# yjb6/SaRO-GS

Measured on AMD Instinct MI355X. Metric: rendered views/s (fwd+bwd) at 1080p vs #Gaussians, higher is better.
Workload: dtype f32; 1 GPU; BASELINE configs[4] stress-1080p: synth(P=3000000, seed 0) SH3, 1920x1080, one view per GPU, fwd+bwd; protocol=SURVEY 8d: 1 / median of per-call device-synchronised wall-clock fwd+bwd, pose_table=off for value (every pose a first visit); on for value_warm, gaussians=3000000, width=1920, height=1080, sh_degree=3, exp_mode=0, poses_per_rank=8, late_gaussians_cold=2255988, word_fork=0

## Files before the change

### include/gsrast.h

```cpp
#ifndef GSRAST_H_INCLUDED
#define GSRAST_H_INCLUDED

#include <stddef.h>
#include <stdint.h>

#ifdef __cplusplus
extern "C" {
#endif

#define GSRAST_ABI_VERSION 6
#define GSRAST_TILE_X 16
#define GSRAST_TILE_Y 16

typedef void* (*gsrast_alloc_fn)(void* ctx, size_t bytes);

int gsrast_forward(gsrast_alloc_fn geometry_alloc, void* geometry_ctx,
                   gsrast_alloc_fn binning_alloc, void* binning_ctx,
                   gsrast_alloc_fn image_alloc, void* image_ctx,
                   int P, int D, int M,
                   const float* background,
                   int width, int height,
                   const float* means3D,
                   const float* shs,
                   const float* colors_precomp,
// ... 66 lines not shown

int gsrast_grad_rows_pack(int P, const unsigned char* touched , float* const* dense, const float* factor , uint32_t* rows, uint32_t cap, void* stream);
int gsrast_grad_rows_clear(int P, const uint32_t* chunks, int n_chunks, size_t chunk_words, uint32_t cap, float* const* dense , int M,
                           float* dL_dsh, float* d_features_dc, float* d_features_rest, void* stream);
int gsrast_grad_rows_add(int P, const uint32_t* chunk, uint32_t cap, float* const* dense, int D, int M, const float* means3D, float scale,
                         float* dL_dsh, float* d_features_dc, float* d_features_rest, void* stream);

int gsrast_debug_export(int P, int R, int width, int height,
                        const char* geom_buffer, const char* binning_buffer, const char* image_buffer,
                        float* depths, float* means2D , float* cov3D ,
                        float* conic_opacity , float* rgb ,
                        unsigned char* clamped , uint32_t* tiles_touched,
                        uint64_t* keys_sorted , uint32_t* point_list ,
                        uint32_t* ranges , float* final_T ,
                        uint32_t* n_contrib , void* stream);

typedef struct gsrast_options {
    int exp_mode;
    int binning;
    int tile_clip;
    int cull;
    int lpt;
    int speculative;
    int fwd_pixels_per_lane;
    int bwd_pixels_per_lane;
    int sh_grad_factors;
    int side_stream;
    int grads_zeroed;
    int backward_phase;
    int depth_sort;
// ... 298 lines not shown
```

### saro-gs_amd/csrc/gsrast_binning.h

```cpp
#pragma once
#include "gsrast_common.h"

namespace gsrast {
#define GSRAST_OCC_ATTR(n) __attribute__((amdgpu_waves_per_eu(n, n)))
#ifdef GSRAST_RSCAT_WAVES
#define GSRAST_RSCAT_OCC GSRAST_OCC_ATTR(GSRAST_RSCAT_WAVES)
#else
#define GSRAST_RSCAT_OCC
#endif
#ifdef GSRAST_BSCAT_WAVES
#define GSRAST_BSCAT_OCC GSRAST_OCC_ATTR(GSRAST_BSCAT_WAVES)
#else
#define GSRAST_BSCAT_OCC
#endif
#ifdef GSRAST_BSORT_WAVES
#define GSRAST_BSORT_OCC GSRAST_OCC_ATTR(GSRAST_BSORT_WAVES)
#else
#define GSRAST_BSORT_OCC
#endif
#ifdef GSRAST_EMIT_WAVES
#define GSRAST_EMIT_OCC GSRAST_OCC_ATTR(GSRAST_EMIT_WAVES)
#else
#define GSRAST_EMIT_OCC
#endif
// ... 772 lines not shown
    uint32_t run = wave_incl_scan(wsum) - wsum;
    const uint32_t wtot = __shfl(run + wsum, 63, 64);
#pragma unroll
    for (int d = 32; d >= 1; d >>= 1) { tsum += __shfl_xor(tsum, d, 64); wall += __shfl_xor(wall, d, 64); }
    uint32_t* scanbuf = reinterpret_cast<uint32_t*>(grp);
    for (uint32_t e = 0; e < E; e++) { const uint32_t t = lane * E + e; if (t < n) { run += aux[t]; scanbuf[t] = run; } }
    wave_sync();
    for (uint32_t t = lane; t < n; t += 64) bwincl[(size_t)b * BK_CAP + t] = scanbuf[t];
    if (lane == 0) {
        if (early_only) { binfo[b] = make_uint4(n, wtot, n_all - n, over); binfo_all[b] = make_uint4(n_all, wall, tsum, over); }
        else binfo[b] = make_uint4(n, wtot, tsum, over);
        bwsum[b] = wtot;
    }
}

__device__ __forceinline__ void depth_bucket_totals(const uint4* __restrict__ binfo, uint32_t nb, uint32_t* __restrict__ scalars,
                                                    uint32_t* host_out = nullptr, uint32_t host_seq = 0,
                                                    const uint4* __restrict__ binfo_e = nullptr )
{
    __shared__ unsigned long long s_t[256];
    __shared__ uint32_t s_q[256], s_qe[256];
    uint32_t over = 0, q = 0, qe = 0;
    unsigned long long tsum = 0;
    for (uint32_t k0 = threadIdx.x; k0 < nb; k0 += 256 * 8) {
        uint4 v[8];
#pragma unroll
        for (int u = 0; u < 8; u++) { const uint32_t k = k0 + u * 256; v[u] = k < nb ? binfo[k] : make_uint4(0u, 0u, 0u, 0u); }
#pragma unroll
        for (int u = 0; u < 8; u++) { q += v[u].y; tsum += v[u].z; over |= v[u].w; }
        if (binfo_e) {
// ... 119 lines not shown
        const uint32_t prev = tile_keys_sorted[i - 1];
        if (cur != prev) { ranges[prev].y = i; ranges[cur].x = i; }
    }
    if (i == R - 1) ranges[cur].y = R;
}

__device__ __forceinline__ double sqrt_newton(double x)
{
    const float xf = (float)x;
    if (!(xf > 1e-30f) || !(xf < 1e30f)) return sqrt(x);
    const float s0f = __builtin_sqrtf(xf);
    const double s0 = (double)s0f;
    return __builtin_fma(__builtin_fma(-s0, s0, x), 0.5 * (double)__builtin_amdgcn_rcpf(s0f), s0);
}

__global__ void __launch_bounds__(256) GSRAST_EMIT_OCC
emit_column_runs_kernel(int P, const uint32_t* __restrict__ order, const uint32_t* __restrict__ woffsets ,
                        const float4* __restrict__ binrec, int W, int H, int cull, uint32_t capQ,
                        uint16_t* __restrict__ run_keys, uint2* __restrict__ run_vals,
                        const uint4* __restrict__ binfo = nullptr, const uint32_t* __restrict__ bwsum = nullptr, uint32_t nbuckets = 0,
                        uint32_t* __restrict__ scalars = nullptr ,
                        uint32_t* __restrict__ host_out = nullptr, uint32_t host_seq = 0 ,
                        const uint4* __restrict__ binfo_all = nullptr, const uint32_t* __restrict__ pred = nullptr,
                        uint32_t* __restrict__ redo_bucket_cnt = nullptr, int n_redo_cnt = 0, HintTable* __restrict__ redo_hints = nullptr,
                        unsigned long long* __restrict__ host_fallback = nullptr, uint32_t host_fb_seq = 0 ,
                        const unsigned char* __restrict__ need2 = nullptr, int gx_tiles = 0, uint32_t* __restrict__ pass2_counts = nullptr,
                        const float4* __restrict__ rec0 = nullptr, const float4* __restrict__ rec1 = nullptr, const uint2* __restrict__ rect = nullptr)
{
    if (pred && *pred == 0u) return;
    __shared__ uint32_t s_e[4][64], s_g[4][64], s_x0[4][64], s_yh[4][64];
    __shared__ double s_det[4][64], s_t2c[4][64], s_invc[4][64], s_dymax[4][64], s_dxtop[4][64];
    __shared__ float s_b[4][64], s_mx[4][64], s_my[4][64];
    __shared__ uint32_t s_mode[4][64];
    if (redo_bucket_cnt && blockIdx.x == nbuckets) {
        for (int i = threadIdx.x; i < n_redo_cnt; i += blockDim.x) redo_bucket_cnt[i] = 0u;
        if (threadIdx.x == 0 && redo_hints) atomicAdd(&redo_hints->cut_fallbacks, 1u);
        uint32_t q2 = 1u;
        if (pass2_counts) {
            unsigned long long* const s_t2 = reinterpret_cast<unsigned long long*>(&s_det[0][0]);
            uint32_t* const s_q2 = &s_e[0][0];
            unsigned long long ts = 0; uint32_t q = 0;
            for (uint32_t k = threadIdx.x; k < nbuckets; k += 256) { const uint4 v = binfo[k]; q += v.y; ts += v.z; }
            s_t2[threadIdx.x] = ts; s_q2[threadIdx.x] = q;
            __syncthreads();
            for (int st = 128; st > 0; st >>= 1) { if ((int)threadIdx.x < st) { s_t2[threadIdx.x] += s_t2[threadIdx.x + st]; s_q2[threadIdx.x] += s_q2[threadIdx.x + st]; } __syncthreads(); }
            if (threadIdx.x == 0) { pass2_counts[0] = (uint32_t)s_t2[0]; pass2_counts[1] = s_q2[0]; pass2_counts[2] = 0u; pass2_counts[3] = (uint32_t)(s_t2[0] >> 32); q2 = s_q2[0] ? s_q2[0] : 1u; }
        }
        if (threadIdx.x == 0 && host_fallback) __hip_atomic_store(host_fallback, ((unsigned long long)host_fb_seq << 32) | (unsigned long long)q2, __ATOMIC_RELAXED, __HIP_MEMORY_SCOPE_SYSTEM);
        return;
    }
    const unsigned lane = lane_id(), wave = threadIdx.x >> 6;
    uint32_t nloc = 0, run0 = 0, nchunks = 1;
    uint32_t pre_g = 0, pre_w = 0, pre_wm = 0;
    if (binfo) {
        __shared__ uint32_t s_run0[4];
        uint32_t part = 0;
        const uint4* w4 = reinterpret_cast<const uint4*>(bwsum);
        if (scalars && blockIdx.x == 0) { depth_bucket_totals(binfo_all ? binfo_all : binfo, nbuckets, scalars, host_out, host_seq, binfo_all ? binfo : nullptr); return; }
        const uint32_t b = scalars ? blockIdx.x - 1u : blockIdx.x, n4 = (b + 3) / 4;
        order += (size_t)b * BK_CAP; woffsets += (size_t)b * BK_CAP;
        pre_g = order[threadIdx.x]; pre_w = woffsets[threadIdx.x]; pre_wm = threadIdx.x ? woffsets[threadIdx.x - 1] : 0u;
        for (uint32_t q0 = threadIdx.x; q0 < n4; q0 += 256 * 8) {
            uint4 v[8];
#pragma unroll
            for (int u = 0; u < 8; u++) { const uint32_t q = q0 + u * 256; v[u] = q < n4 ? w4[q] : make_uint4(0u, 0u, 0u, 0u); }
#pragma unroll
            for (int u = 0; u < 8; u++) {
                const uint32_t k = 4 * (q0 + u * 256);
                part += (k < b ? v[u].x : 0u) + (k + 1 < b ? v[u].y : 0u) + (k + 2 < b ? v[u].z : 0u) + (k + 3 < b ? v[u].w : 0u);
            }
        }
#pragma unroll
        for (int d = 32; d >= 1; d >>= 1) part += __shfl_xor(part, d, 64);
        if (lane == 0) s_run0[wave] = part;
        const uint4 bi = binfo[b];
        __syncthreads();
        run0 = s_run0[0] + s_run0[1] + s_run0[2] + s_run0[3];
        nloc = bi.x; nchunks = (nloc + 255u) / 256u;
        P = (int)nloc;
    }
    for (uint32_t chunk = 0; chunk < nchunks; chunk++) {
    if (chunk) __syncthreads();
    const int j = binfo ? (int)(chunk * 256u + threadIdx.x) : (int)(blockIdx.x * blockDim.x + threadIdx.x);
    uint32_t g = 0, w = 0, incl, x0 = 0, yh = 0;
    if (j < P) {
        const bool pre = binfo && chunk == 0;
        g = pre ? pre_g : order[j];
        incl = run0 + (pre ? pre_w : woffsets[j]);
        const uint32_t prev = j > 0 ? run0 + (pre ? pre_wm : woffsets[j - 1]) : run0;
        w = incl - prev;
        uint2 rc = make_uint2(0u, 0u);
        float4 r0 = make_float4(0.f, 0.f, 0.f, 0.f), r1 = r0;
        if (w != 0u) {
            if (binrec) {
                r0 = binrec[2 * (size_t)g]; r1 = binrec[2 * (size_t)g + 1];
                rc = make_uint2(__float_as_uint(r1.z), __float_as_uint(r1.w));
            } else {
// ... 63 lines not shown
            const int thi = min((int)(y0 + h) - 1, (int)fmin(phi, (double)(H - 1)) >> 4);
            if (empty || phi < 0.0 || plo > (double)(H - 1) || thi < tlo) h = 0;
            else { y0 = (uint32_t)tlo; h = (uint32_t)(thi - tlo + 1); }
            yhv = y0 | (h << 16);
        }
        if (need2 && (yhv >> 16) != 0u) {
            const uint32_t y0 = yhv & 0xFFFFu, h = yhv >> 16;
            bool any = false;
            for (uint32_t yy = y0; yy < y0 + h; yy++) any |= need2[yy * (uint32_t)gx_tiles + x] != 0;
            if (!any) yhv = y0;
        }
        run_keys[wstart + o] = (uint16_t)x;
        run_vals[wstart + o] = make_uint2(s_g[wave][sidx], yhv);
    }
    }
}

__global__ void __launch_bounds__(256)
run_hist_rows_kernel(const uint2* __restrict__ run_vals, uint32_t Q, const uint32_t* __restrict__ Q_dev,
                     uint32_t* __restrict__ block_hist, uint32_t nblk, uint32_t nrows ,
                     const uint32_t* __restrict__ pred = nullptr)
{
    __shared__ int diff[257];
    if (pred && *pred == 0u) return;
    Q = dev_count(Q, Q_dev);
    for (int k = threadIdx.x; k < 257; k += 256) diff[k] = 0;
    __syncthreads();
    const uint32_t r0 = blockIdx.x * RUNS_PER_BLOCK;
    for (uint32_t k = threadIdx.x; k < (uint32_t)RUNS_PER_BLOCK; k += 256) {
        const uint32_t r = r0 + k;
// ... 287 lines not shown
```

### saro-gs_amd/csrc/gsrast_capi.hip

```cpp
#include "gsrast_host.h"
#include "gsrast_common.h"
#include "gsrast_policy.h"
#include "gsrast_preprocess.h"
#include "gsrast_binning.h"
#include "gsrast_blend.h"
#include "gsrast_contrib.h"
#include "gsrast_features.h"
#include "gsrast_distort.h"
#include "gsrast_exchange.h"

#include <algorithm>
#include <atomic>
#include <chrono>
#include <cstdlib>
#include <thread>
#include <cstdio>
#include <cmath>
#include <cstring>
#include <dlfcn.h>
#ifndef GSRAST_LATE_FILL_WGS
#define GSRAST_LATE_FILL_WGS 256
#endif
#include <mutex>
#include <string>
// ... 814 lines not shown
    return v ? fail(GSRAST_E_ARG, "forward: a Gaussian passed as prefiltered was culled by the near plane (the reference traps: auxiliary.h:156-160)") : GSRAST_OK;
}

static const char* raw_inputs_check(int P, int M, const gsrast_raw_inputs* in)
{
    if (!in) return "raw: NULL inputs";
    if (P == 0) return nullptr;
    if (!in->xyz || !in->rotation || !in->scaling || !in->opacity_logit || !in->features_dc || (M > 1 && !in->features_rest)) return "raw: NULL required input";
    if (M < 1 || M * 3 > PP_SH_MAX || ((M * 3) & 3)) return "raw: M must be 4 or 16 (SH rows of a multiple of 16 bytes, at most 16 coefficients)";
    if (((uintptr_t)in->rotation | (uintptr_t)in->features_dc | (uintptr_t)in->features_rest | (uintptr_t)in->shs_res) & 15) return "raw: rotation / features_dc / features_rest / shs_res must be 16-byte aligned";
    return nullptr;
}

extern "C++" { namespace {
struct BucketSortArgs {
    const uint4* slab; const uint32_t* gcount; uint32_t nb; const uint32_t* bkey; uint32_t *border, *bwincl; uint4* binfo; uint32_t* bwsum;
    uint4* binfo_all = nullptr;
    const uint32_t* pred = nullptr; const unsigned long long* keep_bits = nullptr;
    uint32_t* zero_words = nullptr; uint32_t n_zero_words = 0; uint4* zero_quads = nullptr; uint32_t n_zero_quads = 0;
};
void launch_bucket_sort(hipStream_t s, const BucketSortArgs& a)
{
    depth_bucket_sort_kernel<<<(a.nb + BK_WAVES - 1) / BK_WAVES, 64 * BK_WAVES, 0, s>>>(a.slab, a.gcount, a.nb, a.bkey, a.border, a.bwincl, a.binfo, a.bwsum, a.binfo_all, a.pred, a.keep_bits,
                                                                                   a.zero_words, a.n_zero_words, a.zero_quads, a.n_zero_quads);
}
struct EmitArgs {
    uint32_t grid; int P; const uint32_t *order, *woffsets; const float4* binrec; int W, H, clip; uint32_t capQ; uint16_t* run_keys; uint2* run_vals;
    const float4 *rec0, *rec1; const uint2* rect;
    const uint4* binfo = nullptr; const uint32_t* bwsum = nullptr; uint32_t nbuckets = 0;
    uint32_t* scalars = nullptr; uint32_t* host_out = nullptr; uint32_t host_seq = 0;
    const uint4* binfo_all = nullptr; const uint32_t* pred = nullptr;
    uint32_t* redo_bucket_cnt = nullptr; int n_redo_cnt = 0; HintTable* redo_hints = nullptr; unsigned long long* host_fallback = nullptr; uint32_t host_fb_seq = 0;
    const unsigned char* need2 = nullptr; int gx_tiles = 0; uint32_t* pass2_counts = nullptr;
};
void launch_emit(hipStream_t s, const EmitArgs& a)
{
    emit_column_runs_kernel<<<a.grid, 256, 0, s>>>(a.P, a.order, a.woffsets, a.binrec, a.W, a.H, a.clip, a.capQ, a.run_keys, a.run_vals, a.binfo, a.bwsum, a.nbuckets, a.scalars,
                                               a.host_out, a.host_seq, a.binfo_all, a.pred, a.redo_bucket_cnt, a.n_redo_cnt, a.redo_hints, a.host_fallback, a.host_fb_seq,
                                               a.need2, a.gx_tiles, a.pass2_counts, a.rec0, a.rec1, a.rect);
}
bool trace_on() { static const bool on = getenv("GSRAST_TRACE") != nullptr; return on; }

struct ForwardRun {
    gsrast_context* const ctx; const gsrast_forward_call& c; const gsrast_options o; const std::chrono::steady_clock::time_point t_entry; const hipStream_t stream;
    ForwardPlan plan;
    const float *means3D, *shs, *opacities, *scales, *rotations;
    const gsrast_raw_inputs* rawin = nullptr; RawArgs raw{};
    float *out_acc_depth = nullptr, *out_alpha = nullptr;
    int P = 0, W = 0, H = 0; uint32_t T = 0, nbk = 0; CamArgs cam;
    GeomLayout GL; ImgLayout IL; char *geom = nullptr, *img = nullptr, *bin = nullptr; uint32_t cap = 0, capQ = 0;
    float4 *rec0, *rec1, *rec2, *binrec, *grec; uint32_t* tiles; uint2* rect; uint32_t *kA, *kB, *vA, *vB, *offsets, *woffsets, *hist, *scan_tmp, *scalars, *hint_sel, *prefilter_word;
    uint4 *bk_slab, *bk_info, *bk_info_e; uint32_t *bk_count, *bk_key, *bk_order, *bk_wincl, *bk_base, *bk_order_e, *bk_wincl_e, *bk_base_e;
    unsigned long long *color_skip, *cand_bits; unsigned char *untouched = nullptr, *tile_flags; uint32_t* bucket_cnt; uint16_t* bucket_list; uint2* ranges;
    uint32_t *zcut_used = nullptr, *tau_hist = nullptr, *zhist_call = nullptr; TauBins tau_bins{};
    HintTable* hints = nullptr;
    uint32_t zh_klo = 0, zh_wave_mask = 0; int zh_shift = 0;
    bool zhist_ctx = false; int tau_ctx_device = -1;
    struct SideJoinGuard {
        SideStream* side = nullptr; bool launched = false , joined = false;
        ~SideJoinGuard() { if (launched && side && !joined) (void)hipStreamSynchronize(side->stream); }
    } fork;
    bool bucketed = false;
    bool totals_pending = false;
    bool sort_redone = false;
    Readback *rb_pre = nullptr, *rb_flag = nullptr, *rb = nullptr; uint32_t *pre_alias = nullptr, *flag_alias = nullptr; uint32_t pre_seq = 0, flag_seq = 0;
    ChainGate* gate = nullptr; uint32_t gseq = 0, *gdone = nullptr, *gpred = nullptr;
    uint32_t counts[12] = { 0 }; uint32_t nQ1 = 0;
// ... 43 lines not shown
        GL = geom_layout((size_t)P);
        geom = (char*)c.geometry_alloc(c.geometry_ctx, GL.total);
        if (!geom) return fail(GSRAST_E_ALLOC, "forward: geometry allocation failed");
        IL = img_layout((size_t)W, (size_t)H);
        img = (char*)c.image_alloc(c.image_ctx, IL.total);
        if (!img) return fail(GSRAST_E_ALLOC, "forward: image allocation failed");
        rec0 = at<float4>(geom, GL.rec0); rec1 = at<float4>(geom, GL.rec1); rec2 = at<float4>(geom, GL.rec2); grec = at<float4>(geom, GL.grec);
        tiles = at<uint32_t>(geom, GL.tiles); rect = at<uint2>(geom, GL.rect);
        kA = at<uint32_t>(geom, GL.keyA); kB = at<uint32_t>(geom, GL.keyB); vA = at<uint32_t>(geom, GL.valA); vB = at<uint32_t>(geom, GL.valB);
        offsets = at<uint32_t>(geom, GL.offsets); woffsets = at<uint32_t>(geom, GL.woffsets); hist = at<uint32_t>(geom, GL.hist); scan_tmp = at<uint32_t>(geom, GL.scan_tmp);
        scalars = at<uint32_t>(geom, GL.scalars); hint_sel = scalars + HINT_SEL;
        bk_slab = at<uint4>(geom, GL.bk_slab); bk_info = at<uint4>(geom, GL.bk_info); bk_info_e = at<uint4>(geom, GL.bk_info_e);
        bk_count = at<uint32_t>(geom, GL.bk_count); bk_key = at<uint32_t>(geom, GL.bk_key);
        bk_order = at<uint32_t>(geom, GL.bk_order); bk_wincl = at<uint32_t>(geom, GL.bk_wincl); bk_base = at<uint32_t>(geom, GL.bk_base);
        bk_order_e = at<uint32_t>(geom, GL.bk_order_e); bk_wincl_e = at<uint32_t>(geom, GL.bk_wincl_e); bk_base_e = at<uint32_t>(geom, GL.bk_base_e);
        color_skip = at<unsigned long long>(geom, GL.color_skip); cand_bits = at<unsigned long long>(geom, GL.cand_bits);
        tile_flags = at<unsigned char>(img, IL.tile_flags); bucket_cnt = at<uint32_t>(img, IL.bucket_cnt); bucket_list = at<uint16_t>(img, IL.bucket_list);
        ranges = at<uint2>(img, IL.ranges);
        prefilter_word = c.prefiltered ? scalars + SC_PREFILTER : nullptr;
        if (prefilter_word) GS_HIP(hipMemsetAsync(prefilter_word, 0, sizeof(uint32_t), s));
        nbk = depth_buckets_host((size_t)P);
        zh_klo = ctx->zrange.klo.load(); zh_shift = ctx->zrange.shift.load();
        while ((((size_t)P + 63) / 64) / ((size_t)zh_wave_mask + 1) > 1024) zh_wave_mask = 2u * zh_wave_mask + 1u;
        if (o.side_stream) fork.side = side_stream_of(ctx);
        return GSRAST_OK;
    }

    int begin_policy(hipStream_t s)
    {
        hints = plan.want_hints ? hints_of(ctx, T, s) : nullptr;
// ... 72 lines not shown
                P, means3D, scales, rotations, opacities, raw, c.cov3D_precomp, cam, c.radii, rec0, rec1, cov_dbg,
                tiles, rect, binrec, kA, plan.bucket_sort ? nullptr : vA, plan.clip ? 1 : 0, bucket_cnt, zhist_call, zh_klo, zh_shift, zh_wave_mask, bk_count, nzero, hints, hint_sel,
                zcut_used, T, scalars, host_found, pre_seq, prefilter_word, untouched, tau_hist, tau_bins);
        }); });
        GS_LAUNCHED("preprocess_fwd");
        ctx->last_prologue_ns = (uint32_t)std::min<long long>(std::chrono::duration_cast<std::chrono::nanoseconds>(std::chrono::steady_clock::now() - t_entry).count(), 0xFFFFFFFFll);
        if (tau_hist) {
            const dim3 tg((unsigned)((cam.gx + TAU_TILE - 1) / TAU_TILE), (unsigned)((cam.gy + TAU_TILE - 1) / TAU_TILE));
            tau_cut_kernel<<<tg, TAU_BLK * TAU_BLK, 0, s>>>(tau_hist, T, cam.gx, cam.gy, tau_bins, (uint32_t)ctx->pol.tau_req.load() * 256u, hints ? hint_sel : nullptr, plan.tau_forced ? 1 : 0,
                                              zcut_used, tau_bins.scale > 0.0f ? 0 : 1);
            GS_LAUNCHED("tau_cut");
        }
        return GSRAST_OK;
    }

    BucketSortArgs whole_buckets() const { return BucketSortArgs{ bk_slab, bk_count, nbk, bk_key, bk_order, bk_wincl, bk_info, bk_base }; }
    int sort_and_scan(hipStream_t s, bool assume, bool buckets)
    {
        bucketed = buckets; totals_pending = false;
        if (buckets) {
            ProfScope ps(K_SORT_DEPTH, s);
            const int items = depth_scatter_items((size_t)P);
            const bool two = plan.two_level;
            auto scatter = two ? (items == BK_ITEMS_WIDE ? depth_bucket_scatter_kernel<BK_ITEMS_WIDE, true> : depth_bucket_scatter_kernel<BK_ITEMS, true>)
                               : (items == BK_ITEMS_WIDE ? depth_bucket_scatter_kernel<BK_ITEMS_WIDE, false> : depth_bucket_scatter_kernel<BK_ITEMS, false>);
            uint4* cslab = reinterpret_cast<uint4*>(grec);
            const uint32_t ccap = depth_coarse_cap((size_t)P, nbk);
            uint32_t* gccount = at<uint32_t>(geom, GL.bk_ccount);
            scatter<<<(P + 256 * items - 1) / (256 * items), 256, 0, s>>>(kA, rect, tiles, (uint32_t)P, zhist_call, zh_klo, zh_shift, nbk, two ? gccount : bk_count, two ? cslab : bk_slab, bk_key, scalars + SC_ZBINS,
                                                                           zcut_used, T, (uint32_t)cam.gx, scalars + SC_N_LATE, plan.cut ? color_skip : nullptr, (uint32_t)plan.cut_cs, ccap);
            GS_LAUNCHED("depth_bucket_scatter");
            if (two) {
                depth_bucket_refine_kernel<<<(nbk >> BK_CSHIFT) * BK_XCD, 256, 0, s>>>(cslab, gccount, nbk, bk_count, bk_slab, ccap);
                GS_LAUNCHED("depth_bucket_refine");
            }
            BucketSortArgs a = whole_buckets();
            if (plan.cut) { a.border = bk_order_e; a.bwincl = bk_wincl_e; a.binfo = bk_info_e; a.bwsum = bk_base_e; a.binfo_all = bk_info; }
            a.zero_words = zhist_ctx ? zhist_call : nullptr; a.n_zero_words = ZH_COPIES * ZH_BINS;
            if (tau_ctx_device >= 0) { a.zero_quads = reinterpret_cast<uint4*>(tau_hist); a.n_zero_quads = (uint32_t)((size_t)TAU_COPIES * T * TAU_BINS / 4); }
            launch_bucket_sort(s, a);
            GS_LAUNCHED("depth_bucket_sort");
            if (a.zero_quads) { std::lock_guard<std::mutex> lk(ctx->mu); ctx->tau_dev_dirty[tau_ctx_device] = false; }
            totals_pending = true;
            return GSRAST_OK;
        }
        {   ProfScope ps(K_SORT_DEPTH, s);
            if (plan.bucket_sort) {
                iota_kernel<<<(P + 255) / 256, 256, 0, s>>>(vA, (uint32_t)P);
                GS_LAUNCHED("iota");
            }
            const SortAdapt<uint32_t, uint32_t> ad{ at<uint32_t>(geom, GL.keyC), at<uint32_t>(geom, GL.valC), at<uint32_t>(geom, GL.sort_minmax), scalars + 8, assume };
            int rc = radix_sort<uint32_t, uint32_t, GSRAST_DEPTH_ITEMS>(kA, vA, kB, vB, (uint32_t)P, 32, hist, scan_tmp, s, rect, plan.runbin ? nullptr : offsets, woffsets, nullptr, &ad);
// ... 77 lines not shown
            }
        }
        return GSRAST_OK;
    }

    int run_binning(hipStream_t s, uint32_t nQ, const uint32_t* counts_dev, int mode, const uint32_t* pred, bool readback_after_emit)
    {
        const RunBinLayout RL = runbin_layout((size_t)cap, (size_t)capQ);
        uint16_t *rkA = at<uint16_t>(bin, RL.rkeyA), *rkB = at<uint16_t>(bin, RL.rkeyB);
        uint2 *rvA = at<uint2>(bin, RL.rvalA), *rvB = at<uint2>(bin, RL.rvalB);
        uint32_t *hist_x = at<uint32_t>(bin, RL.hist_x), *hist_y = at<uint32_t>(bin, RL.hist_y), *rscan = at<uint32_t>(bin, RL.scan_tmp), *plist_w = at<uint32_t>(bin, RL.point_list);
        const uint32_t* Q_dev = counts_dev ? counts_dev + 1 : nullptr;
        const int xbits = tile_bits((size_t)cam.gx);
        {   ProfScope ps(K_EMIT, s);
            EmitArgs e{};
            e.grid = nbk + 1; e.P = P; e.order = bk_order; e.woffsets = bk_wincl; e.binrec = binrec; e.W = W; e.H = H; e.clip = o.tile_clip; e.capQ = capQ; e.run_keys = rkA; e.run_vals = rvA;
            e.rec0 = rec0; e.rec1 = rec1; e.rect = rect;
            if (bucketed) { e.binfo = bk_info; e.bwsum = bk_base; e.nbuckets = nbk; }
            if (bucketed && mode == 1) {
                e.order = bk_order_e; e.woffsets = bk_wincl_e; e.binfo = bk_info_e; e.bwsum = bk_base_e; e.binfo_all = bk_info;
                e.scalars = scalars; e.host_out = flag_alias; e.host_seq = flag_seq;
            } else if (bucketed && mode == 2) {
                BucketSortArgs a = whole_buckets(); a.pred = pred; a.keep_bits = cand_bits;
                launch_bucket_sort(s, a);
                e.pred = pred; e.redo_bucket_cnt = bucket_cnt; e.n_redo_cnt = XCD_GROUPS * WORK_BUCKETS ; e.redo_hints = hints;
                e.host_fallback = rb_pre ? reinterpret_cast<unsigned long long*>(pre_alias) + RB_FALLBACK : nullptr; e.host_fb_seq = pre_seq;
                e.need2 = tile_flags; e.gx_tiles = cam.gx; e.pass2_counts = scalars + SC_PASS2;
            } else if (bucketed) {
                if (plan.cut) {
                    launch_bucket_sort(s, whole_buckets());
                    GS_LAUNCHED("depth_bucket_sort");
                }
                e.scalars = scalars; e.host_out = flag_alias; e.host_seq = flag_seq;
            } else { e.grid = (uint32_t)((P + 255) / 256); e.order = vA; e.woffsets = woffsets; }
            launch_emit(s, e);
// ... 831 lines not shown
    GS_LAUNCHED("export_geom");
    if (R > 0 && binning_buffer && image_buffer && (keys_sorted || point_list)) {
        export_keys_kernel<<<T, 256, 0, s>>>(at<uint2>(image_buffer, IL.ranges), at<uint32_t>(binning_buffer, 0),
                                             at<float4>(geom_buffer, GL.rec1), keys_sorted, point_list, (uint32_t)R);
        GS_LAUNCHED("export_keys");
    }
    if (image_buffer) {
        const size_t N = (size_t)width * height;
        if (ranges) GS_HIP(hipMemcpyAsync(ranges, image_buffer + IL.ranges, (size_t)T * 8, hipMemcpyDeviceToDevice, s));
        if (final_T) GS_HIP(hipMemcpyAsync(final_T, image_buffer + IL.final_T, N * 4, hipMemcpyDeviceToDevice, s));
        if (n_contrib) GS_HIP(hipMemcpyAsync(n_contrib, image_buffer + IL.n_contrib, N * 4, hipMemcpyDeviceToDevice, s));
    }
    return GSRAST_OK;
}

}

#ifdef GSRAST_SCATTER_TIMING
extern "C" int gsrast_debug_scatter_timing(unsigned long long* out, int reset)
{
    if (hipMemcpyFromSymbol(out, HIP_SYMBOL(gsrast::g_scat), sizeof(unsigned long long) * 16) != hipSuccess) return -1;
    if (reset) { unsigned long long z[16] = {0}; z[14] = ~0ull; if (hipMemcpyToSymbol(HIP_SYMBOL(gsrast::g_scat), z, sizeof(z)) != hipSuccess) return -1; }
    return 0;
}
#endif
#if defined(GSRAST_DEBUG_COUNTERS) || defined(GSRAST_DEBUG_TIMING)
extern "C" int gsrast_debug_counters(unsigned long long* out, int reset)
{
    if (hipMemcpyFromSymbol(out, HIP_SYMBOL(gsrast::g_dbg), sizeof(unsigned long long) * 16) != hipSuccess) return -1;
    if (reset) { unsigned long long z[16] = {0}; z[11] = ~0ull ; if (hipMemcpyToSymbol(HIP_SYMBOL(gsrast::g_dbg), z, sizeof(z)) != hipSuccess) return -1; }
// ... 4 lines not shown
```

### saro-gs_amd/csrc/gsrast_common.h

```cpp
#pragma once
#include <hip/hip_runtime.h>
#include "gsrast_host.h"
#include <stdint.h>
#include <stddef.h>

namespace gsrast {

constexpr int TILE_X = 16;
constexpr int TILE_Y = 16;
constexpr int TILE_PIX = TILE_X * TILE_Y;
constexpr int WAVE = 64;

#ifndef GSRAST_REC_STRIDE
#define GSRAST_REC_STRIDE 1
#endif
constexpr int REC_STRIDE = GSRAST_REC_STRIDE;
struct GeomLayout {
    size_t rec0, rec1, rec2, cov3D, clamped, tiles, rect, binrec, keyA, keyB, valA, valB, offsets, woffsets,
        hist, scan_tmp, scalars, grec, keyC, valC, sort_minmax, shdA, shdB, shdC, zhist, bk_key, bk_count, bk_ccount , bk_slab, bk_order, bk_wincl, bk_info, bk_base,
        bk_order_e, bk_wincl_e, bk_info_e, bk_base_e ,
        color_skip ,
        cand_bits ,
        skip2 ,
        untouched , total;
};
constexpr int GREC = 16;
constexpr size_t BUCKET_SORT_MIN_P = 32768;
#ifndef GSRAST_BK_TARGET
#define GSRAST_BK_TARGET 256
#endif
#ifndef GSRAST_BK_CAP
#define GSRAST_BK_CAP 1024
#endif
constexpr int ZH_BINS = 1024, ZH_COPIES = 8 ;
constexpr int ZH_TAIL = 64, ZH_MID = ZH_BINS - 2 * ZH_TAIL, ZH_TAIL_LOG = 4;
constexpr uint32_t ZH_KLO_DEFAULT = 0x3E400000u;
constexpr int ZH_SHIFT_DEFAULT = 21;
constexpr uint32_t ZH_KEY_TOP = 0x7F800000u;
__host__ __device__ inline void zh_locate(uint32_t key, uint32_t kmid, int shift, uint32_t& bin, uint32_t& pos, int& wlog)
{
    const int d = (int)key - (int)kmid;
    const int wt = shift + ZH_TAIL_LOG;
// ... 124 lines not shown
    L.scan_tmp = c.take(st * 4);
    L.scalars = c.take(256);
    L.grec = c.take(Pp * GREC * 4);
    L.keyC = c.take(Pp * 4); L.valC = c.take(Pp * 4);
    L.sort_minmax = c.take(2 * rs_blocks_n(Pp, GSRAST_DEPTH_ITEMS) * 4);
    L.shdA = c.take(Pp * 16); L.shdB = c.take(Pp * 16); L.shdC = c.take(Pp * 4);
    L.zhist = c.take(ZH_COPIES * ZH_BINS * 4);
    {
        const size_t nb = Pp >= BUCKET_SORT_MIN_P ? depth_buckets_host(Pp) : 0;
        L.bk_count = c.take(nb * 8 * 4);
        L.bk_ccount = c.take(8 * 256 * 4);
        L.bk_slab = c.take(nb * GSRAST_BK_CAP * 16);
        L.bk_order = c.take(nb * GSRAST_BK_CAP * 4); L.bk_wincl = c.take(nb * GSRAST_BK_CAP * 4);
        L.bk_info = c.take(nb * 16); L.bk_base = c.take(nb * 4); L.bk_key = c.take((nb + 1) * 4);
        L.bk_order_e = c.take(nb * GSRAST_BK_CAP * 4); L.bk_wincl_e = c.take(nb * GSRAST_BK_CAP * 4); L.bk_info_e = c.take(nb * 16); L.bk_base_e = c.take(nb * 4);
    }
    L.color_skip = c.take(((Pp + 63) / 64) * 8 + 256);
    L.cand_bits = c.take(((Pp + 63) / 64) * 8 + 256);
    L.skip2 = c.take(((Pp + 63) / 64) * 8 + 256);
    L.untouched = c.take(Pp + 256);
    L.total = c.o + 256;
    return L;
}
static inline BinLayout bin_layout(size_t R)
{
    BinLayout L; Carver c;
    size_t Rp = R ? R : 1;
    L.valA = c.take(Rp * 4); L.valB = c.take(Rp * 4); L.keyA = c.take(Rp * 4); L.keyB = c.take(Rp * 4);
    size_t hist_n = 256 * rs_blocks(Rp);
    L.hist = c.take(hist_n * 4);
// ... 197 lines not shown
```

### saro-gs_amd/diff_gaussian_rasterization_ch3/_C.py

```python
from __future__ import annotations

import ctypes as C
import itertools
import os
import threading
from typing import List, Optional, Tuple

import torch

_HERE = os.path.dirname(os.path.abspath(__file__))
LIB_PATH = os.path.join(_HERE, "libgsrast_hip.so")

NUM_CHANNELS = 3
ABI_VERSION = 6

_ALLOC_FN = C.CFUNCTYPE(C.c_void_p, C.c_void_p, C.c_size_t)
_lib: Optional[C.CDLL] = None

RENDER_AUX = 0x1
RENDER_ANTIALIAS = 0x2
RENDER_ABSGRAD = 0x4
RENDER_POSEGRAD = 0x8
FAMILY_DENSE, FAMILY_RAW = 0, 1
FEATURES_MAX_C = 64
# ... 111 lines not shown
_opt, _adam, _dens, _mlp, _bila, _plane = (C.POINTER(S) for S in (OptionsStruct, AdamGroupStruct, DensifyGroupStruct, Mlp3Struct, BilagridStruct, PlaneStruct))
_vpp, _uints = C.POINTER(_vp), C.POINTER(C.c_uint)

SIGNATURES = {
    "gsrast_forward": (_ci, (_ALLOC_FN, _vp, _ALLOC_FN, _vp, _ALLOC_FN, _vp, _ci, _ci, _ci, _vp, _ci, _ci, _vp, _vp, _vp, _vp, _vp, _cf, _vp, _vp, _vp, _vp, _vp, _cf, _cf, _ci, _vp, _vp, _vp, _vp)),
    "gsrast_backward": (_ci, (_ci, _ci, _ci, _ci, _vp, _ci, _ci, _vp, _vp, _vp, _vp, _cf, _vp, _vp, _vp, _vp, _vp, _cf, _cf) + (_vp,) * 15),
    "gsrast_render_forward": (_ci, (_vp, _opt, C.POINTER(ForwardCallStruct))),
    "gsrast_render_backward": (_ci, (_opt, C.POINTER(BackwardCallStruct))),
    "gsrast_mark_visible": (_ci, (_ci, _vp, _vp, _vp, _vp, _vp)),
    "gsrast_geometry_bytes": (_sz, (_ci,)),
    "gsrast_binning_bytes": (_sz, (_ci, _ci, _ci)),
    "gsrast_image_bytes": (_sz, (_ci, _ci)),
    "gsrast_pose_scratch_bytes": (_sz, (_ci,)),
    "gsrast_alloc_prealloc": (_vp, (_vp, _sz)),
    "gsrast_debug_export": (_ci, (_ci, _ci, _ci, _ci) + (_vp,) * 16),
    "gsrast_options_init": (None, (_opt,)),
    "gsrast_context_create": (_vp, ()),
    "gsrast_context_destroy": (None, (_vp,)),
    "gsrast_context_query": (_ci, (_vp, _str)),
    "gsrast_policy_event": (_ci, (_vp, _str, _ci, _ci, _ci)),
    "gsrast_debug_forward_plan": (_ci, (_vp, _opt, C.c_uint, _ci, _ci, _ci, C.POINTER(_ci))),
    "gsrast_debug_backward_plan": (_ci, (_opt, C.c_uint, C.POINTER(_ci), C.POINTER(_ci))),
    "gsrast_set_option": (_ci, (_str, _ci)),
    "gsrast_get_option": (_ci, (_str,)),
    "gsrast_profile_kernel_count": (_ci, ()),
    "gsrast_profile_kernel_name": (_str, (_ci,)),
    "gsrast_profile_collect": (_ci, ()),
    "gsrast_profile_read": (_ci, (_ci, C.POINTER(_cd), C.POINTER(_ll))),
    "gsrast_profile_reset": (None, ()),
    "gsrast_last_error": (_str, ()),
# ... 944 lines not shown
        clamped=torch.zeros((P, 3), dtype=torch.uint8, device=dev),
        tiles_touched=torch.zeros(P, dtype=torch.int32, device=dev),
        keys_sorted=torch.zeros(max(R, 1), dtype=torch.int64, device=dev)[:R],
        point_list=torch.zeros(max(R, 1), dtype=torch.int32, device=dev)[:R],
        ranges=torch.zeros((T, 2), dtype=torch.int32, device=dev),
        final_T=torch.zeros((H, W), **f32), n_contrib=torch.zeros((H, W), dtype=torch.int32, device=dev))
    keep_cov = int(lib().gsrast_get_option(b"debug_state")) != 0
    if not keep_cov:
        del out["cov3D"]
    launch("gsrast_debug_export", dev, P, R, W, H, _ptr(geomBuffer), _ptr(binningBuffer), _ptr(imageBuffer), out["depths"].data_ptr(),
         out["means2D"].data_ptr(), out["cov3D"].data_ptr() if keep_cov else None, out["conic_opacity"].data_ptr(),
         out["rgb"].data_ptr(), out["clamped"].data_ptr(), out["tiles_touched"].data_ptr(),
         _ptr(out["keys_sorted"]), _ptr(out["point_list"]), out["ranges"].data_ptr(),
         out["final_T"].data_ptr(), out["n_contrib"].data_ptr())
    return out
```

Baseline: 808.7 views/s.

## Precompute bucket run prefixes and compact live buckets for persistent emit workers

Adds a single-block prefix kernel after the depth-bucket sort. It turns the per-bucket run counts into an exclusive prefix and writes a compacted list of non-empty buckets. The emit kernel no longer recomputes each bucket's run offset with a per-block scan over all earlier buckets. It now runs a capped grid of persistent workers that loop over only the live buckets, which removes quadratic prefix work and idle blocks for empty buckets. The cost is an extra kernel launch with a serial chunk loop, plus extra syncs inside the worker loop, and it adds a debug export entry point.

```diff
diff --git a/include/gsrast.h b/include/gsrast.h
--- a/include/gsrast.h
+++ b/include/gsrast.h
@@ -104,6 +104,9 @@
                         uint64_t* keys_sorted , uint32_t* point_list ,
                         uint32_t* ranges , float* final_T ,
                         uint32_t* n_contrib , void* stream);
+
+int gsrast_debug_export_buckets(int P, const char* geom_buffer, int early, uint32_t* counts , uint32_t* first_run ,
+                                uint32_t* live , void* stream);
 
 typedef struct gsrast_options {
     int exp_mode;
diff --git a/saro-gs_amd/csrc/gsrast_binning.h b/saro-gs_amd/csrc/gsrast_binning.h
--- a/saro-gs_amd/csrc/gsrast_binning.h
+++ b/saro-gs_amd/csrc/gsrast_binning.h
@@ -810,6 +810,50 @@
     }
 }
 
+constexpr int BK_PFX_THREADS = 1024, BK_PFX_CHUNKS = BK_MAX_BUCKETS / 256;
+__global__ void __launch_bounds__(BK_PFX_THREADS)
+depth_bucket_prefix_kernel(uint32_t* __restrict__ bwsum, uint32_t nb , uint32_t* __restrict__ live,
+                           const uint32_t* __restrict__ pred )
+{
+    __shared__ uint32_t s_w[BK_PFX_CHUNKS], s_c[BK_PFX_CHUNKS];
+    if (pred && *pred == 0u) return;
+    const unsigned lane = lane_id(), wave = threadIdx.x >> 6;
+    constexpr int WAVES = BK_PFX_THREADS / 64, PER = BK_PFX_CHUNKS / WAVES;
+    const uint32_t nchunks = nb / 256u;
+    uint4 v[PER]; uint32_t si[PER], ci[PER], s[PER], c[PER];
+#pragma unroll
+    for (int u = 0; u < PER; u++) {
+        const uint32_t ch = wave + (uint32_t)u * WAVES;
+        v[u] = ch < nchunks ? reinterpret_cast<const uint4*>(bwsum)[ch * 64u + lane] : make_uint4(0u, 0u, 0u, 0u);
+    }
+#pragma unroll
+    for (int u = 0; u < PER; u++) {
+        const uint32_t ch = wave + (uint32_t)u * WAVES;
+        s[u] = v[u].x + v[u].y + v[u].z + v[u].w;
+        c[u] = (v[u].x ? 1u : 0u) + (v[u].y ? 1u : 0u) + (v[u].z ? 1u : 0u) + (v[u].w ? 1u : 0u);
+        si[u] = wave_incl_scan(s[u]); ci[u] = wave_incl_scan(c[u]);
+        if (lane == 63 && ch < (uint32_t)BK_PFX_CHUNKS) { s_w[ch] = si[u]; s_c[ch] = ci[u]; }
+    }
+    __syncthreads();
+    uint32_t nlive = 0;
+    for (uint32_t k = 0; k < nchunks; k++) nlive += s_c[k];
+#pragma unroll
+    for (int u = 0; u < PER; u++) {
+        const uint32_t ch = wave + (uint32_t)u * WAVES;
+        if (ch >= nchunks) continue;
+        uint32_t base = si[u] - s[u], at = ci[u] - c[u];
+        for (uint32_t k = 0; k < ch; k++) { base += s_w[k]; at += s_c[k]; }
+        const uint32_t b0 = ch * 256u + 4u * lane;
+        reinterpret_cast<uint4*>(bwsum)[ch * 64u + lane] = make_uint4(base, base + v[u].x, base + v[u].x + v[u].y, base + v[u].x + v[u].y + v[u].z);
+        if (v[u].x) live[at++] = b0;
+        if (v[u].y) live[at++] = b0 + 1u;
+        if (v[u].z) live[at++] = b0 + 2u;
+        if (v[u].w) live[at] = b0 + 3u;
+    }
+    for (uint32_t k = nlive + threadIdx.x; k < nb; k += BK_PFX_THREADS) live[k] = BK_NO_BUCKET;
+    if (threadIdx.x == 0) live[nb] = nlive;
+}
+
 __device__ __forceinline__ void depth_bucket_totals(const uint4* __restrict__ binfo, uint32_t nb, uint32_t* __restrict__ scalars,
                                                     uint32_t* host_out = nullptr, uint32_t host_seq = 0,
                                                     const uint4* __restrict__ binfo_e = nullptr )
@@ -959,11 +1003,16 @@
     return __builtin_fma(__builtin_fma(-s0, s0, x), 0.5 * (double)__builtin_amdgcn_rcpf(s0f), s0);
 }
 
+#ifndef GSRAST_EMIT_WORKERS
+#define GSRAST_EMIT_WORKERS 2048
+#endif
+__host__ __device__ inline uint32_t emit_workers(uint32_t nb) { return nb < (uint32_t)GSRAST_EMIT_WORKERS ? nb : (uint32_t)GSRAST_EMIT_WORKERS; }
+
 __global__ void __launch_bounds__(256) GSRAST_EMIT_OCC
 emit_column_runs_kernel(int P, const uint32_t* __restrict__ order, const uint32_t* __restrict__ woffsets ,
                         const float4* __restrict__ binrec, int W, int H, int cull, uint32_t capQ,
                         uint16_t* __restrict__ run_keys, uint2* __restrict__ run_vals,
-                        const uint4* __restrict__ binfo = nullptr, const uint32_t* __restrict__ bwsum = nullptr, uint32_t nbuckets = 0,
+                        const uint4* __restrict__ binfo = nullptr, const uint32_t* __restrict__ brun0 = nullptr, const uint32_t* __restrict__ live = nullptr, uint32_t nbuckets = 0,
                         uint32_t* __restrict__ scalars = nullptr ,
                         uint32_t* __restrict__ host_out = nullptr, uint32_t host_seq = 0 ,
                         const uint4* __restrict__ binfo_all = nullptr, const uint32_t* __restrict__ pred = nullptr,
@@ -977,7 +1026,7 @@
     __shared__ double s_det[4][64], s_t2c[4][64], s_invc[4][64], s_dymax[4][64], s_dxtop[4][64];
     __shared__ float s_b[4][64], s_mx[4][64], s_my[4][64];
     __shared__ uint32_t s_mode[4][64];
-    if (redo_bucket_cnt && blockIdx.x == nbuckets) {
+    if (redo_bucket_cnt && blockIdx.x == gridDim.x - 1u) {
         for (int i = threadIdx.x; i < n_redo_cnt; i += blockDim.x) redo_bucket_cnt[i] = 0u;
         if (threadIdx.x == 0 && redo_hints) atomicAdd(&redo_hints->cut_fallbacks, 1u);
         uint32_t q2 = 1u;
@@ -995,37 +1044,32 @@
         return;
     }
     const unsigned lane = lane_id(), wave = threadIdx.x >> 6;
+    const uint32_t* const order0 = order; const uint32_t* const woffsets0 = woffsets;
+    uint32_t nworkers = 1, li = 0, b_next = BK_NO_BUCKET;
+    if (binfo) {
+        if (scalars && blockIdx.x == 0) { depth_bucket_totals(binfo_all ? binfo_all : binfo, nbuckets, scalars, host_out, host_seq, binfo_all ? binfo : nullptr); return; }
+        const uint32_t first = scalars ? 1u : 0u;
+        nworkers = gridDim.x - first - (redo_bucket_cnt ? 1u : 0u);
+        li = blockIdx.x - first;
+        b_next = li < nbuckets ? live[li] : BK_NO_BUCKET;
+    }
+    for (bool first_bucket = true; ; first_bucket = false) {
     uint32_t nloc = 0, run0 = 0, nchunks = 1;
     uint32_t pre_g = 0, pre_w = 0, pre_wm = 0;
     if (binfo) {
-        __shared__ uint32_t s_run0[4];
-        uint32_t part = 0;
-        const uint4* w4 = reinterpret_cast<const uint4*>(bwsum);
-        if (scalars && blockIdx.x == 0) { depth_bucket_totals(binfo_all ? binfo_all : binfo, nbuckets, scalars, host_out, host_seq, binfo_all ? binfo : nullptr); return; }
-        const uint32_t b = scalars ? blockIdx.x - 1u : blockIdx.x, n4 = (b + 3) / 4;
-        order += (size_t)b * BK_CAP; woffsets += (size_t)b * BK_CAP;
+        const uint32_t b = b_next;
+        if (b == BK_NO_BUCKET) break;
+        order = order0 + (size_t)b * BK_CAP; woffsets = woffsets0 + (size_t)b * BK_CAP;
         pre_g = order[threadIdx.x]; pre_w = woffsets[threadIdx.x]; pre_wm = threadIdx.x ? woffsets[threadIdx.x - 1] : 0u;
-        for (uint32_t q0 = threadIdx.x; q0 < n4; q0 += 256 * 8) {
-            uint4 v[8];
-#pragma unroll
-            for (int u = 0; u < 8; u++) { const uint32_t q = q0 + u * 256; v[u] = q < n4 ? w4[q] : make_uint4(0u, 0u, 0u, 0u); }
-#pragma unroll
-            for (int u = 0; u < 8; u++) {
-                const uint32_t k = 4 * (q0 + u * 256);
-                part += (k < b ? v[u].x : 0u) + (k + 1 < b ? v[u].y : 0u) + (k + 2 < b ? v[u].z : 0u) + (k + 3 < b ? v[u].w : 0u);
-            }
-        }
-#pragma unroll
-        for (int d = 32; d >= 1; d >>= 1) part += __shfl_xor(part, d, 64);
-        if (lane == 0) s_run0[wave] = part;
         const uint4 bi = binfo[b];
-        __syncthreads();
-        run0 = s_run0[0] + s_run0[1] + s_run0[2] + s_run0[3];
+        run0 = brun0[b];
+        li += nworkers;
+        b_next = li < nbuckets ? live[li] : BK_NO_BUCKET;
         nloc = bi.x; nchunks = (nloc + 255u) / 256u;
         P = (int)nloc;
-    }
+    } else if (!first_bucket) break;
     for (uint32_t chunk = 0; chunk < nchunks; chunk++) {
-    if (chunk) __syncthreads();
+    if (chunk || !first_bucket) __syncthreads();
     const int j = binfo ? (int)(chunk * 256u + threadIdx.x) : (int)(blockIdx.x * blockDim.x + threadIdx.x);
     uint32_t g = 0, w = 0, incl, x0 = 0, yh = 0;
     if (j < P) {
@@ -1119,6 +1163,7 @@
         run_vals[wstart + o] = make_uint2(s_g[wave][sidx], yhv);
     }
     }
+    }
 }
 
 __global__ void __launch_bounds__(256)
diff --git a/saro-gs_amd/csrc/gsrast_capi.hip b/saro-gs_amd/csrc/gsrast_capi.hip
--- a/saro-gs_amd/csrc/gsrast_capi.hip
+++ b/saro-gs_amd/csrc/gsrast_capi.hip
@@ -852,7 +852,7 @@
 
 extern "C++" { namespace {
 struct BucketSortArgs {
-    const uint4* slab; const uint32_t* gcount; uint32_t nb; const uint32_t* bkey; uint32_t *border, *bwincl; uint4* binfo; uint32_t* bwsum;
+    const uint4* slab; const uint32_t* gcount; uint32_t nb; const uint32_t* bkey; uint32_t *border, *bwincl; uint4* binfo; uint32_t *bwsum, *live;
     uint4* binfo_all = nullptr;
     const uint32_t* pred = nullptr; const unsigned long long* keep_bits = nullptr;
     uint32_t* zero_words = nullptr; uint32_t n_zero_words = 0; uint4* zero_quads = nullptr; uint32_t n_zero_quads = 0;
@@ -861,11 +861,12 @@
 {
     depth_bucket_sort_kernel<<<(a.nb + BK_WAVES - 1) / BK_WAVES, 64 * BK_WAVES, 0, s>>>(a.slab, a.gcount, a.nb, a.bkey, a.border, a.bwincl, a.binfo, a.bwsum, a.binfo_all, a.pred, a.keep_bits,
                                                                                    a.zero_words, a.n_zero_words, a.zero_quads, a.n_zero_quads);
+    depth_bucket_prefix_kernel<<<1, BK_PFX_THREADS, 0, s>>>(a.bwsum, a.nb, a.live, a.pred);
 }
 struct EmitArgs {
     uint32_t grid; int P; const uint32_t *order, *woffsets; const float4* binrec; int W, H, clip; uint32_t capQ; uint16_t* run_keys; uint2* run_vals;
     const float4 *rec0, *rec1; const uint2* rect;
-    const uint4* binfo = nullptr; const uint32_t* bwsum = nullptr; uint32_t nbuckets = 0;
+    const uint4* binfo = nullptr; const uint32_t* brun0 = nullptr; const uint32_t* live = nullptr; uint32_t nbuckets = 0;
     uint32_t* scalars = nullptr; uint32_t* host_out = nullptr; uint32_t host_seq = 0;
     const uint4* binfo_all = nullptr; const uint32_t* pred = nullptr;
     uint32_t* redo_bucket_cnt = nullptr; int n_redo_cnt = 0; HintTable* redo_hints = nullptr; unsigned long long* host_fallback = nullptr; uint32_t host_fb_seq = 0;
@@ -873,7 +874,7 @@
 };
 void launch_emit(hipStream_t s, const EmitArgs& a)
 {
-    emit_column_runs_kernel<<<a.grid, 256, 0, s>>>(a.P, a.order, a.woffsets, a.binrec, a.W, a.H, a.clip, a.capQ, a.run_keys, a.run_vals, a.binfo, a.bwsum, a.nbuckets, a.scalars,
+    emit_column_runs_kernel<<<a.grid, 256, 0, s>>>(a.P, a.order, a.woffsets, a.binrec, a.W, a.H, a.clip, a.capQ, a.run_keys, a.run_vals, a.binfo, a.brun0, a.live, a.nbuckets, a.scalars,
                                                a.host_out, a.host_seq, a.binfo_all, a.pred, a.redo_bucket_cnt, a.n_redo_cnt, a.redo_hints, a.host_fallback, a.host_fb_seq,
                                                a.need2, a.gx_tiles, a.pass2_counts, a.rec0, a.rec1, a.rect);
 }
@@ -888,7 +889,7 @@
     int P = 0, W = 0, H = 0; uint32_t T = 0, nbk = 0; CamArgs cam;
     GeomLayout GL; ImgLayout IL; char *geom = nullptr, *img = nullptr, *bin = nullptr; uint32_t cap = 0, capQ = 0;
     float4 *rec0, *rec1, *rec2, *binrec, *grec; uint32_t* tiles; uint2* rect; uint32_t *kA, *kB, *vA, *vB, *offsets, *woffsets, *hist, *scan_tmp, *scalars, *hint_sel, *prefilter_word;
-    uint4 *bk_slab, *bk_info, *bk_info_e; uint32_t *bk_count, *bk_key, *bk_order, *bk_wincl, *bk_base, *bk_order_e, *bk_wincl_e, *bk_base_e;
+    uint4 *bk_slab, *bk_info, *bk_info_e; uint32_t *bk_count, *bk_key, *bk_order, *bk_wincl, *bk_base, *bk_order_e, *bk_wincl_e, *bk_base_e, *bk_live, *bk_live_e;
     unsigned long long *color_skip, *cand_bits; unsigned char *untouched = nullptr, *tile_flags; uint32_t* bucket_cnt; uint16_t* bucket_list; uint2* ranges;
     uint32_t *zcut_used = nullptr, *tau_hist = nullptr, *zhist_call = nullptr; TauBins tau_bins{};
     HintTable* hints = nullptr;
@@ -962,6 +963,7 @@
         bk_count = at<uint32_t>(geom, GL.bk_count); bk_key = at<uint32_t>(geom, GL.bk_key);
         bk_order = at<uint32_t>(geom, GL.bk_order); bk_wincl = at<uint32_t>(geom, GL.bk_wincl); bk_base = at<uint32_t>(geom, GL.bk_base);
         bk_order_e = at<uint32_t>(geom, GL.bk_order_e); bk_wincl_e = at<uint32_t>(geom, GL.bk_wincl_e); bk_base_e = at<uint32_t>(geom, GL.bk_base_e);
+        bk_live = at<uint32_t>(geom, GL.bk_live); bk_live_e = at<uint32_t>(geom, GL.bk_live_e);
         color_skip = at<unsigned long long>(geom, GL.color_skip); cand_bits = at<unsigned long long>(geom, GL.cand_bits);
         tile_flags = at<unsigned char>(img, IL.tile_flags); bucket_cnt = at<uint32_t>(img, IL.bucket_cnt); bucket_list = at<uint16_t>(img, IL.bucket_list);
         ranges = at<uint2>(img, IL.ranges);
@@ -1064,7 +1066,7 @@
         return GSRAST_OK;
     }
 
-    BucketSortArgs whole_buckets() const { return BucketSortArgs{ bk_slab, bk_count, nbk, bk_key, bk_order, bk_wincl, bk_info, bk_base }; }
+    BucketSortArgs whole_buckets() const { return BucketSortArgs{ bk_slab, bk_count, nbk, bk_key, bk_order, bk_wincl, bk_info, bk_base, bk_live }; }
     int sort_and_scan(hipStream_t s, bool assume, bool buckets)
     {
         bucketed = buckets; totals_pending = false;
@@ -1085,7 +1087,7 @@
                 GS_LAUNCHED("depth_bucket_refine");
             }
             BucketSortArgs a = whole_buckets();
-            if (plan.cut) { a.border = bk_order_e; a.bwincl = bk_wincl_e; a.binfo = bk_info_e; a.bwsum = bk_base_e; a.binfo_all = bk_info; }
+            if (plan.cut) { a.border = bk_order_e; a.bwincl = bk_wincl_e; a.binfo = bk_info_e; a.bwsum = bk_base_e; a.live = bk_live_e; a.binfo_all = bk_info; }
             a.zero_words = zhist_ctx ? zhist_call : nullptr; a.n_zero_words = ZH_COPIES * ZH_BINS;
             if (tau_ctx_device >= 0) { a.zero_quads = reinterpret_cast<uint4*>(tau_hist); a.n_zero_quads = (uint32_t)((size_t)TAU_COPIES * T * TAU_BINS / 4); }
             launch_bucket_sort(s, a);
@@ -1193,11 +1195,11 @@
         const int xbits = tile_bits((size_t)cam.gx);
         {   ProfScope ps(K_EMIT, s);
             EmitArgs e{};
-            e.grid = nbk + 1; e.P = P; e.order = bk_order; e.woffsets = bk_wincl; e.binrec = binrec; e.W = W; e.H = H; e.clip = o.tile_clip; e.capQ = capQ; e.run_keys = rkA; e.run_vals = rvA;
+            e.grid = emit_workers(nbk) + 1; e.P = P; e.order = bk_order; e.woffsets = bk_wincl; e.binrec = binrec; e.W = W; e.H = H; e.clip = o.tile_clip; e.capQ = capQ; e.run_keys = rkA; e.run_vals = rvA;
             e.rec0 = rec0; e.rec1 = rec1; e.rect = rect;
-            if (bucketed) { e.binfo = bk_info; e.bwsum = bk_base; e.nbuckets = nbk; }
+            if (bucketed) { e.binfo = bk_info; e.brun0 = bk_base; e.live = bk_live; e.nbuckets = nbk; }
             if (bucketed && mode == 1) {
-                e.order = bk_order_e; e.woffsets = bk_wincl_e; e.binfo = bk_info_e; e.bwsum = bk_base_e; e.binfo_all = bk_info;
+                e.order = bk_order_e; e.woffsets = bk_wincl_e; e.binfo = bk_info_e; e.brun0 = bk_base_e; e.live = bk_live_e; e.binfo_all = bk_info;
                 e.scalars = scalars; e.host_out = flag_alias; e.host_seq = flag_seq;
             } else if (bucketed && mode == 2) {
                 BucketSortArgs a = whole_buckets(); a.pred = pred; a.keep_bits = cand_bits;
@@ -2059,6 +2061,19 @@
     return GSRAST_OK;
 }
 
+int gsrast_debug_export_buckets(int P, const char* geom_buffer, int early, uint32_t* counts, uint32_t* first_run, uint32_t* live, void* stream)
+{
+    hipStream_t s = (hipStream_t)stream;
+    if (P <= 0 || !geom_buffer) return fail(GSRAST_E_ARG, "debug_export_buckets: bad arguments");
+    if ((size_t)P < BUCKET_SORT_MIN_P) return 0;
+    const GeomLayout GL = geom_layout((size_t)P);
+    const size_t nb = depth_buckets_host((size_t)P);
+    if (counts) GS_HIP(hipMemcpy2DAsync(counts, 4, geom_buffer + (early ? GL.bk_info_e : GL.bk_info), 16, 4, nb, hipMemcpyDeviceToDevice, s));
+    if (first_run) GS_HIP(hipMemcpyAsync(first_run, geom_buffer + (early ? GL.bk_base_e : GL.bk_base), nb * 4, hipMemcpyDeviceToDevice, s));
+    if (live) GS_HIP(hipMemcpyAsync(live, geom_buffer + (early ? GL.bk_live_e : GL.bk_live), (nb + 1) * 4, hipMemcpyDeviceToDevice, s));
+    return (int)nb;
+}
+
 }
 
 #ifdef GSRAST_SCATTER_TIMING
diff --git a/saro-gs_amd/csrc/gsrast_common.h b/saro-gs_amd/csrc/gsrast_common.h
--- a/saro-gs_amd/csrc/gsrast_common.h
+++ b/saro-gs_amd/csrc/gsrast_common.h
@@ -19,6 +19,7 @@
     size_t rec0, rec1, rec2, cov3D, clamped, tiles, rect, binrec, keyA, keyB, valA, valB, offsets, woffsets,
         hist, scan_tmp, scalars, grec, keyC, valC, sort_minmax, shdA, shdB, shdC, zhist, bk_key, bk_count, bk_ccount , bk_slab, bk_order, bk_wincl, bk_info, bk_base,
         bk_order_e, bk_wincl_e, bk_info_e, bk_base_e ,
+        bk_live, bk_live_e ,
         color_skip ,
         cand_bits ,
         skip2 ,
@@ -26,6 +27,7 @@
 };
 constexpr int GREC = 16;
 constexpr size_t BUCKET_SORT_MIN_P = 32768;
+constexpr uint32_t BK_NO_BUCKET = 0xFFFFFFFFu;
 #ifndef GSRAST_BK_TARGET
 #define GSRAST_BK_TARGET 256
 #endif
@@ -180,6 +182,7 @@
         L.bk_order = c.take(nb * GSRAST_BK_CAP * 4); L.bk_wincl = c.take(nb * GSRAST_BK_CAP * 4);
         L.bk_info = c.take(nb * 16); L.bk_base = c.take(nb * 4); L.bk_key = c.take((nb + 1) * 4);
         L.bk_order_e = c.take(nb * GSRAST_BK_CAP * 4); L.bk_wincl_e = c.take(nb * GSRAST_BK_CAP * 4); L.bk_info_e = c.take(nb * 16); L.bk_base_e = c.take(nb * 4);
+        L.bk_live = c.take((nb + 1) * 4); L.bk_live_e = c.take((nb + 1) * 4);
     }
     L.color_skip = c.take(((Pp + 63) / 64) * 8 + 256);
     L.cand_bits = c.take(((Pp + 63) / 64) * 8 + 256);
diff --git a/saro-gs_amd/diff_gaussian_rasterization_ch3/_C.py b/saro-gs_amd/diff_gaussian_rasterization_ch3/_C.py
--- a/saro-gs_amd/diff_gaussian_rasterization_ch3/_C.py
+++ b/saro-gs_amd/diff_gaussian_rasterization_ch3/_C.py
@@ -149,6 +149,7 @@
     "gsrast_pose_scratch_bytes": (_sz, (_ci,)),
     "gsrast_alloc_prealloc": (_vp, (_vp, _sz)),
     "gsrast_debug_export": (_ci, (_ci, _ci, _ci, _ci) + (_vp,) * 16),
+    "gsrast_debug_export_buckets": (_ci, (_ci, _vp, _ci, _vp, _vp, _vp, _vp)),
     "gsrast_options_init": (None, (_opt,)),
     "gsrast_context_create": (_vp, ()),
     "gsrast_context_destroy": (None, (_vp,)),
@@ -1123,3 +1124,18 @@
          _ptr(out["keys_sorted"]), _ptr(out["point_list"]), out["ranges"].data_ptr(),
          out["final_T"].data_ptr(), out["n_contrib"].data_ptr())
     return out
+
+
+def debug_export_buckets(P: int, geomBuffer, early: bool) -> Optional[dict]:
+    dev = geomBuffer.device
+    cap = 8192
+    buf = torch.zeros((3, cap + 1), dtype=torch.int32, device=dev)
+    with _on_device(dev):
+        nb = int(lib().gsrast_debug_export_buckets(P, _ptr(geomBuffer), 1 if early else 0, buf[0].data_ptr(), buf[1].data_ptr(), buf[2].data_ptr(), _stream_of(dev)))
+    if nb < 0:
+        raise _err(nb, "gsrast_debug_export_buckets")
+    if nb == 0:
+        return None
+    host = buf.cpu().numpy().view("uint32")
+    n_live = int(host[2, nb])
+    return dict(nb=nb, counts=host[0, :nb].copy(), first_run=host[1, :nb].copy(), live=host[2, :n_live].copy(), live_tail=host[2, n_live:nb].copy())
```

New measurement: 799.7 views/s. 0.989x the previous value.
